# javieryu/nn_distributed_training

Measured on NVIDIA H100. Metric: consensus node-rounds/sec (DiNNO, dist_mnist_PAPER; rounds/sec x graph nodes), higher is better.
Workload: dtype fp64

## Files before the change

### nn_distributed_training_b200/ops/csrc/mnist_cl64.cu

```cuda
#include "mnist_device.cuh"

namespace nndt {
namespace mnist {

namespace cl64 {

constexpr int NT = 512, CL = 4, CELLS = 36, KC = 108, WS = 116, HS = 68;
constexpr int PXR = 10 * HW;
constexpr int KT = (KC + 7) / 8;
constexpr int HR = 68;
NNDT_DEVINL int hr(int j) { return (j >> 4) * 17 + (j & 15); }
constexpr int PART_WC = 0, PART_BC = 75, PART_B1 = 78, PART_W2 = 142, PART_B2 = 782, PART_LOSS = 792, PART_N = 793;

template <int MS>
struct Smem {
  static constexpr int NO = MS / CL;
  static constexpr bool kDoublePix = MS <= 32;
  static constexpr int PXS = kDoublePix ? PXR + 2 : PXR;
  double w[HID * WS];
  double a[MS * WS];
  double h[MS * HS];
  alignas(16) unsigned char img[kDoublePix ? MS * PXS * 8 : MS * PXS];
  double lut[kDoublePix ? 1 : 256];
  double h_loc[NO * HR > CL * 80 ? NO * HR : CL * 80];
  double dh_loc[NO * HID];
  double part[800];
  double w2[NCLS * HR];
  alignas(16) double b1[HID];
  alignas(16) double b2[16];
  double wc[80];
  double dz[NO * 16];
  double red[NO];
  int sidx[MS];
  int label[MS];
  float valid[MS];
  unsigned char arg[MS * KC];
};
static_assert(sizeof(Smem<16>) <= 227 * 1024 && sizeof(Smem<32>) <= 227 * 1024 && sizeof(Smem<64>) <= 227 * 1024,
              "shared memory budget");

NNDT_DEVINL double wmax(double v) {
#pragma unroll
  for (int o = 16; o > 0; o >>= 1) v = fmax(v, __shfl_xor_sync(0xffffffffu, v, o));
  return v;
}
template <int H>
NNDT_DEVINL void fold_half(double (&v)[16], int lane) {
  const bool up = (lane & (2 * H)) != 0;
#pragma unroll
  for (int i = 0; i < H; ++i) {
    const double send = up ? v[i] : v[i + H], keep = up ? v[i + H] : v[i];
    v[i] = keep + __shfl_xor_sync(0xffffffffu, send, 2 * H);
  }
}
NNDT_DEVINL void warp_reduce_scatter16(double (&v)[16], int lane) {
  fold_half<8>(v, lane); fold_half<4>(v, lane); fold_half<2>(v, lane); fold_half<1>(v, lane);
  v[0] += __shfl_xor_sync(0xffffffffu, v[0], 1);
}
NNDT_DEVINL void dmma_nv(double (&c)[4], double a0, double a1, double b) {
  asm("mma.sync.aligned.m16n8k4.row.col.f64.f64.f64.f64 {%0,%1,%2,%3}, {%4,%5}, {%6}, {%0,%1,%2,%3};"
      : "+d"(c[0]), "+d"(c[1]), "+d"(c[2]), "+d"(c[3])
      : "d"(a0), "d"(a1), "d"(b));
}
template <int NJ, int K, class FA, class FB>
NNDT_DEVINL void gemm_k(double (&c)[NJ][4], int m0, int n0, int lane, FA A, FB B) {
  static_assert(K % 4 == 0, "k steps of 4");
  const int g = lane >> 2, t = lane & 3;
  double a0 = A(m0 + g, t), a1 = A(m0 + g + 8, t), b[NJ];
#pragma unroll
  for (int j = 0; j < NJ; ++j) b[j] = B(t, n0 + 8 * j + g);
#pragma unroll
  for (int k0 = 0; k0 < K; k0 += 4) {
    double na0 = 0.0, na1 = 0.0, nb[NJ];
    if (k0 + 4 < K) {
      const int k = k0 + 4 + t;
      na0 = A(m0 + g, k); na1 = A(m0 + g + 8, k);
#pragma unroll
      for (int j = 0; j < NJ; ++j) nb[j] = B(k, n0 + 8 * j + g);
    }
#pragma unroll
    for (int j = 0; j < NJ; ++j) dmma_nv(c[j], a0, a1, b[j]);
    if (k0 + 4 < K) {
      a0 = na0; a1 = na1;
#pragma unroll
      for (int j = 0; j < NJ; ++j) b[j] = nb[j];
    }
  }
}
NNDT_DEVINL void stamp(long long* prof, int idx, int tid) {
  if (prof != nullptr && tid == 0) {
    long long t;
    asm volatile("mov.u64 %0, %%globaltimer;" : "=l"(t));
    prof[idx] = t;
  }
}

template <int MS>
__global__ void __cluster_dims__(CL, 1, 1) __launch_bounds__(NT, 1)
mnist_cl64_train_kernel(const Args a, const GenericShape gs) {
  using SM = Smem<MS>;
  constexpr int NO = SM::NO, PXS = SM::PXS;
  constexpr bool kDoublePix = SM::kDoublePix;
  static_assert(MS % 16 == 0 && NO <= NT / 32, "tile geometry");
  static_assert(CELLS % 2 == 0 && NCLS % 2 == 0 && 32 + NCLS / 2 <= NT, "16-byte parameter copies");
  extern __shared__ __align__(16) unsigned char smem_raw[];
  SM& sm = *reinterpret_cast<SM*>(smem_raw);
  const int tid = threadIdx.x, warp = tid >> 5, lane = tid & 31;
  const int l = blockIdx.z, bsplit = blockIdx.y, nsplit = gridDim.y;
  const int c = (int)cluster_rank();
  const double* th = reinterpret_cast<const double*>(a.theta) + (size_t)l * a.n_pad;
  const double pmean = gs.mean, pis = gs.inv_std;
  const bool u8 = a.x_is_u8 != 0;
  double* imgd = reinterpret_cast<double*>(sm.img);
  auto pix = [&](int s, int p) -> double {
    if constexpr (kDoublePix) return imgd[s * PXS + p];
    else if (u8) return sm.lut[sm.img[s * PXR + p]];
    else return (double)__ldg(reinterpret_cast<const float*>(a.x) + (size_t)sm.sidx[s] * 784 + 6 * HW * c + p);
  };
  long long* prof = a.prof != nullptr ? a.prof + ((l * nsplit + bsplit) * CL + c) * 64 : nullptr;
  stamp(prof, 0, tid);

  const int call = a.calls != nullptr ? a.calls[l] : 0;
  const BatchGeom bg = batch_geom<true>(a, l, call);
  if (tid < MS) {
    int idx = 0, lab = 0; float ok = 0.f;
    const uint32_t t = (uint32_t)(bsplit * MS + tid);
    if (t < bg.bs) {
      ok = 1.f;
      idx = a.direct ? (int)(l * a.batch + t) : bg.shard_off + (int)feistel_permute(bg.start + t, bg.m, bg.key);
      lab = (int)a.y[idx];
    }
    sm.sidx[tid] = idx; sm.valid[tid] = ok; sm.label[tid] = lab;
  }
  if constexpr (!kDoublePix)
    if (tid < 256) sm.lut[tid] = ((double)tid * (1.0 / 255.0) - pmean) * pis;
  __syncthreads();
  constexpr int NU8 = (MS * 35 + NT - 1) / NT, NF4 = kDoublePix ? (MS * 70 + NT - 1) / NT : 1;
  uint2 pu[NU8]; float4 pf[NF4];
  if (u8) {
#pragma unroll
    for (int i = 0; i < NU8; ++i) {
      const int o = tid + i * NT;
      pu[i] = make_uint2(0, 0);
      if (o < MS * 35) {
        const int s = o / 35, q = o - s * 35;
        if (sm.valid[s] != 0.f)
          pu[i] = *reinterpret_cast<const uint2*>(reinterpret_cast<const unsigned char*>(a.x) + (size_t)sm.sidx[s] * 784 + 6 * HW * c + 8 * q);
      }
    }
  } else if constexpr (kDoublePix) {
#pragma unroll
    for (int i = 0; i < NF4; ++i) {
      const int o = tid + i * NT;
      pf[i] = make_float4(0.f, 0.f, 0.f, 0.f);
      if (o < MS * 70) {
        const int s = o / 70, q = o - s * 70;
        if (sm.valid[s] != 0.f)
          pf[i] = *reinterpret_cast<const float4*>(reinterpret_cast<const float*>(a.x) + (size_t)sm.sidx[s] * 784 + 6 * HW * c + 4 * q);
      }
    }
  }
  if (u8) {
#pragma unroll
    for (int i = 0; i < NU8; ++i) {
      const int o = tid + i * NT;
      if (o < MS * 35) {
        const int s = o / 35, q = o - s * 35;
        if constexpr (kDoublePix) {
          const uint32_t w[2] = {pu[i].x, pu[i].y};
          double* dst = imgd + s * PXS + 8 * q;
#pragma unroll
          for (int j = 0; j < 8; ++j) dst[j] = ((double)((w[j >> 2] >> (8 * (j & 3))) & 0xff) * (1.0 / 255.0) - pmean) * pis;
        } else {
          *reinterpret_cast<uint2*>(sm.img + s * PXR + 8 * q) = pu[i];
        }
      }
    }
  } else if constexpr (kDoublePix) {
#pragma unroll
    for (int i = 0; i < NF4; ++i) {
      const int o = tid + i * NT;
      if (o < MS * 70) {
        double* dst = imgd + (o / 70) * PXS + 4 * (o % 70);
        dst[0] = pf[i].x; dst[1] = pf[i].y; dst[2] = pf[i].z; dst[3] = pf[i].w;
      }
    }
  }
  stamp(prof, 1, tid);
  pdl_wait();
  pdl_launch_dependents();
  stamp(prof, 2, tid);

  constexpr int NW2 = (NCLS * HID + NT - 1) / NT;
  double wcv = 0.0, w2v[NW2];
  if (tid < 75) wcv = __ldcg(th + a.off_wc + tid);
  else if (tid < 78) wcv = __ldcg(th + a.off_bc + (tid - 75));
#pragma unroll
  for (int i = 0; i < NW2; ++i) {
    const int o = tid + i * NT;
    w2v[i] = o < NCLS * HID ? __ldcg(th + a.off_w2 + o) : 0.0;
  }
  for (int o = tid; o < HID * KC / 2; o += NT) {
    const int j = o / (KC / 2), r = o - j * (KC / 2), ch = r / (CELLS / 2), q = 2 * (r - ch * (CELLS / 2));
    cp_async16(sm.w + j * WS + ch * CELLS + q, th + a.off_w1 + (size_t)j * FC1_IN + ch * NPOOL + CELLS * c + q);
  }
  if (tid < HID / 2) cp_async16(sm.b1 + 2 * tid, th + a.off_b1 + 2 * tid);
  else if (tid >= 32 && tid < 32 + NCLS / 2) cp_async16(sm.b2 + 2 * (tid - 32), th + a.off_b2 + 2 * (tid - 32));
  cp_async_commit();
  if (tid < 78) sm.wc[tid] = wcv;
#pragma unroll
  for (int i = 0; i < NW2; ++i) {
    const int o = tid + i * NT;
    if (o < NCLS * HID) sm.w2[(o / HID) * HR + hr(o % HID)] = w2v[i];
  }
  __syncthreads();
  stamp(prof, 3, tid);

  for (int it = tid; it < MS * CELLS; it += NT) {
    const int s = it / CELLS, cell = it - s * CELLS;
    const int pr = cell / PHW, px = cell - pr * PHW;
    const int p0 = (2 * pr) * HW + 2 * px;
    double patch[6][6];
    if constexpr (kDoublePix) {
      const double* src = imgd + s * PXS + p0;
#pragma unroll
      for (int r = 0; r < 6; ++r)
#pragma unroll
        for (int q = 0; q < 6; q += 2) {
          const double2 v = *reinterpret_cast<const double2*>(src + r * HW + q);
          patch[r][q] = v.x; patch[r][q + 1] = v.y;
        }
    } else {
#pragma unroll
      for (int r = 0; r < 6; ++r)
#pragma unroll
        for (int q = 0; q < 6; ++q) patch[r][q] = pix(s, p0 + r * HW + q);
    }
    const bool ok = sm.valid[s] != 0.f;
#pragma unroll 1
    for (int ch = 0; ch < F; ++ch) {
      double a00 = 0, a01 = 0, a10 = 0, a11 = 0;
#pragma unroll
      for (int ky = 0; ky < KS; ++ky)
#pragma unroll
        for (int kx = 0; kx < KS; ++kx) {
          const double w = sm.wc[ch * 25 + ky * 5 + kx];
          a00 += w * patch[ky][kx]; a01 += w * patch[ky][kx + 1];
          a10 += w * patch[ky + 1][kx]; a11 += w * patch[ky + 1][kx + 1];
        }
      double m = a00; int ai = 0;
      if (a01 > m) { m = a01; ai = 1; }
      if (a10 > m) { m = a10; ai = 2; }
      if (a11 > m) { m = a11; ai = 3; }
      m += sm.wc[75 + ch];
      m = (ok && m > 0.0) ? m : 0.0;
      sm.a[s * WS + ch * CELLS + cell] = m;
      sm.arg[s * KC + ch * CELLS + cell] = (unsigned char)(ai | (m > 0.0 ? 4 : 0));
    }
  }
  cp_async_wait<0>();
  __syncthreads();
  stamp(prof, 4, tid);

  {
    constexpr int NJ1 = MS == 64 ? 2 : 1, NGRP = 8 / NJ1;
    if (warp < (MS / 16) * NGRP) {
      const int m0 = 16 * (warp / NGRP), n0 = 8 * NJ1 * (warp % NGRP);
      double acc[NJ1][4];
      zero(acc);
      gemm_k<NJ1, KC>(acc, m0, n0, lane, at(sm.a, WS), at_t(sm.w, WS));
#pragma unroll
      for (int j = 0; j < NJ1; ++j)
#pragma unroll
        for (int i = 0; i < 4; ++i) sm.h[frow(m0, lane, i) * HS + fcol(n0 + 8 * j, lane, i)] = acc[j][i];
    }
  }
  stamp(prof, 5, tid);
  cluster_sync();
  stamp(prof, 6, tid);
  if (c == 0 && tid == 0 && a.calls != nullptr) {
    if (a.arrive == nullptr || nsplit == 1) a.calls[l] = call + 1;
    else if (atomicAdd(a.arrive + l, 1u) == (unsigned)nsplit - 1) { a.arrive[l] = 0; a.calls[l] = call + 1; }
  }

  const int s0 = c * NO;
  const double inv_bs = 1.0 / (double)(bg.bs ? bg.bs : 1);
  if (warp < NO) {
    const int sl = warp, s = s0 + sl;
    double hv[2];
#pragma unroll
    for (int q = 0; q < 2; ++q) {
      const int j = lane + 32 * q;
      const double* src = sm.h + s * HS + j;
      double v = sm.b1[j];
#pragma unroll
      for (int r = 0; r < CL; ++r) v += ld_dsmem(map_to(src, (uint32_t)r));
      hv[q] = v > 0.0 ? v : 0.0;
      sm.h_loc[sl * HR + hr(j)] = hv[q];
    }
    __syncwarp();
    double zp[2];
#pragma unroll
    for (int r = 0; r < 2; ++r) {
      const int o = lane + 32 * r, cc = o >> 2, part = o & 3;
      double v = 0.0;
      if (o < 4 * NCLS) {
#pragma unroll
        for (int jj = 0; jj < 16; ++jj) v += sm.h_loc[sl * HR + part * 17 + jj] * sm.w2[cc * HR + part * 17 + jj];
      }
      v += __shfl_xor_sync(0xffffffffu, v, 1);
      v += __shfl_xor_sync(0xffffffffu, v, 2);
      zp[r] = v;
    }
    static_assert(NCLS > 8 && NCLS <= 16, "two rounds of four lanes per class");
    const double z0 = __shfl_sync(0xffffffffu, zp[0], (4 * lane) & 31), z1 = __shfl_sync(0xffffffffu, zp[1], (4 * lane) & 31);
    const bool cls = lane < NCLS;
    const double zc = cls ? (lane < 8 ? z0 : z1) + sm.b2[lane] : -1.0e300;
    const double mx = wmax(zc);
    const double se = warp_sum(cls ? exp(zc - mx) : 0.0);
    const double lse = mx + log(se);
    const int y = sm.label[s];
    const double ok = (double)sm.valid[s];
    const double dzc = cls ? ok * inv_bs * (exp(zc - lse) - (lane == y ? 1.0 : 0.0)) : 0.0;
    if (cls) sm.dz[sl * 16 + lane] = dzc;
    if (lane == y) sm.red[sl] = ok * (lse - zc);
    double dh[2] = {0.0, 0.0};
#pragma unroll
    for (int cc = 0; cc < NCLS; ++cc) {
      const double d = __shfl_sync(0xffffffffu, dzc, cc);
      dh[0] += d * sm.w2[cc * HR + hr(lane)];
      dh[1] += d * sm.w2[cc * HR + hr(lane + 32)];
    }
#pragma unroll
    for (int q = 0; q < 2; ++q) sm.dh_loc[sl * HID + lane + 32 * q] = hv[q] > 0.0 ? dh[q] : 0.0;
  }
  __syncthreads();
  for (int o = tid; o < NCLS * HID; o += NT) {
    const int cc = o >> 6, j = o & 63;
    double v = 0.0;
    for (int sl = 0; sl < NO; ++sl) v += sm.dz[sl * 16 + cc] * sm.h_loc[sl * HR + hr(j)];
    sm.part[PART_W2 + o] = v;
  }
  if (tid < HID) {
    double v = 0.0;
    for (int sl = 0; sl < NO; ++sl) v += sm.dh_loc[sl * HID + tid];
    sm.part[PART_B1 + tid] = v;
  } else if (tid >= 64 && tid < 64 + NCLS) {
    double v = 0.0;
    for (int sl = 0; sl < NO; ++sl) v += sm.dz[sl * 16 + (tid - 64)];
    sm.part[PART_B2 + (tid - 64)] = v;
  } else if (tid == 96) {
    double v = 0.0;
    for (int sl = 0; sl < NO; ++sl) v += sm.red[sl];
    sm.part[PART_LOSS] = v * inv_bs;
  }
  stamp(prof, 7, tid);
  cluster_sync();
  stamp(prof, 8, tid);
  double* gp = reinterpret_cast<double*>(a.grad_part) + ((size_t)l * nsplit + bsplit) * a.n_pad;
  {
    constexpr int NE = PART_N - PART_B1, PER = (NE + CL - 1) / CL;
    const int o = PART_B1 + c * PER + tid;
    if (tid < PER && o < PART_N) {
      double v = 0.0;
#pragma unroll
      for (int r = 0; r < CL; ++r) v += ld_dsmem(map_to(sm.part + o, (uint32_t)r));
      if (o < PART_W2) gp[a.off_b1 + (o - PART_B1)] = v;
      else if (o < PART_B2) gp[a.off_w2 + (o - PART_W2)] = v;
      else if (o < PART_LOSS) gp[a.off_b2 + (o - PART_B2)] = v;
      else {
        a.loss_part[l * nsplit + bsplit] = (float)v;
        if (a.loss_mirror != nullptr) a.loss_mirror[l * nsplit + bsplit] = (float)v;
      }
    }
  }
  for (int o = tid; o < MS * HID; o += NT) {
    const int s = o >> 6, j = o & 63, r = s / NO;
    sm.h[s * HS + j] = ld_dsmem(map_to(sm.dh_loc + (s - r * NO) * HID + j, (uint32_t)r));
  }
  __syncthreads();
  stamp(prof, 9, tid);

  constexpr int NP2 = (MS / 16) * (KT / 2), NR2 = (NP2 + NT / 32 - 1) / (NT / 32);
  static_assert(KT % 2 == 0 && KC * MS + (NT / 32) * 16 <= HID * WS, "da1 and the conv-grad warp sums fit in the W slice");
  double acc2[NR2][2][4];
#pragma unroll
  for (int r = 0; r < NR2; ++r) {
    zero(acc2[r]);
    const int p = warp + r * (NT / 32);
    if (p < NP2) gemm_k<2, HID>(acc2[r], 16 * (p / (KT / 2)), 16 * (p % (KT / 2)), lane, at(sm.h, HS), at(sm.w, WS));
  }
  __syncthreads();
  stamp(prof, 10, tid);
  double* da1 = sm.w;
#pragma unroll
  for (int r = 0; r < NR2; ++r) {
    const int p = warp + r * (NT / 32);
    if (p < NP2) {
      const int m0 = 16 * (p / (KT / 2)), n0 = 16 * (p % (KT / 2));
#pragma unroll
      for (int jt = 0; jt < 2; ++jt)
#pragma unroll
        for (int i = 0; i < 4; ++i) {
          const int s = frow(m0, lane, i), k = fcol(n0 + 8 * jt, lane, i);
          if (k < KC) da1[k * MS + s] = (sm.arg[s * KC + k] & 4) ? acc2[r][jt][i] : 0.0;
        }
    }
  }
  __syncthreads();
  stamp(prof, 11, tid);
  constexpr int W3 = NT / 32 - HID / 16, NJ3 = KT / 2;
  if (warp >= W3) {
    const int m0 = 16 * (warp - W3);
#pragma unroll 1
    for (int n0 = 0; n0 < 8 * KT; n0 += 8 * NJ3) {
      double acc[NJ3][4];
      zero(acc);
      gemm_k<NJ3, MS>(acc, m0, n0, lane, at_t(sm.h, HS), at(sm.a, WS));
#pragma unroll
      for (int jt = 0; jt < NJ3; ++jt)
#pragma unroll
        for (int i = 0; i < 4; i += 2) {
          const int j = frow(m0, lane, i), k = fcol(n0 + 8 * jt, lane, i);
          if (k < KC) {
            const int ch = k / CELLS, cell = k - ch * CELLS;
            __stcg(reinterpret_cast<double2*>(gp + a.off_w1 + (size_t)j * FC1_IN + ch * NPOOL + CELLS * c + cell),
                   make_double2(acc[jt][i], acc[jt][i + 1]));
          }
        }
    }
    stamp(prof, 12, tid - W3 * 32);
  }
  constexpr int KW = 3, NRUN = MS * 3;
  static_assert(KS * KW < NT / 32 && F * KS <= 16, "conv-grad work split");
  double* wsums = sm.w + KC * MS;
  auto pix2 = [&](int s, int p) -> double2 {
    if constexpr (kDoublePix) return *reinterpret_cast<const double2*>(imgd + s * PXS + p);
    else return make_double2(pix(s, p), pix(s, p + 1));
  };
  if (warp < KS * KW) {
    const int ky = warp / KW;
    double acc[16];
#pragma unroll
    for (int i = 0; i < 16; ++i) acc[i] = 0.0;
#pragma unroll 1
    for (int r = tid - ky * KW * 32; r < NRUN; r += KW * 32) {
      const int s = r % MS, pr = r / MS;
      const int rb = (2 * pr + ky) * HW;
      double x0[6], x1[6];
#pragma unroll
      for (int px = 0; px < PHW; ++px) {
        const int p = rb + 2 * px;
        if (px == 0) {
#pragma unroll
          for (int q = 0; q < 6; q += 2) {
            const double2 u = pix2(s, p + q), v = pix2(s, p + HW + q);
            x0[q] = u.x; x0[q + 1] = u.y; x1[q] = v.x; x1[q + 1] = v.y;
          }
        } else {
#pragma unroll
          for (int q = 0; q < 4; ++q) { x0[q] = x0[q + 2]; x1[q] = x1[q + 2]; }
          const double2 u = pix2(s, p + 4), v = pix2(s, p + HW + 4);
          x0[4] = u.x; x0[5] = u.y; x1[4] = v.x; x1[5] = v.y;
        }
#pragma unroll
        for (int ch = 0; ch < F; ++ch) {
          const int k = ch * CELLS + pr * PHW + px;
          const double g = da1[k * MS + s];
          const int ai = sm.arg[s * KC + k] & 3;
          const double g00 = ai == 0 ? g : 0.0, g01 = ai == 1 ? g : 0.0, g10 = ai == 2 ? g : 0.0, g11 = ai == 3 ? g : 0.0;
#pragma unroll
          for (int kx = 0; kx < KS; ++kx) {
            double& t = acc[ch * KS + kx];
            t = fma(g00, x0[kx], t); t = fma(g01, x0[kx + 1], t);
            t = fma(g10, x1[kx], t); t = fma(g11, x1[kx + 1], t);
          }
        }
      }
    }
    warp_reduce_scatter16(acc, lane);
    if ((lane & 1) == 0 && (lane >> 1) < F * KS) wsums[warp * 16 + (lane >> 1)] = acc[0];
  } else if (warp == KS * KW) {
#pragma unroll 1
    for (int ch = 0; ch < F; ++ch) {
      double v = 0.0;
      for (int o = lane; o < CELLS * MS; o += 32) v += da1[ch * CELLS * MS + o];
      v = warp_sum(v);
      if (lane == 0) wsums[warp * 16 + ch] = v;
    }
  }
  __syncthreads();
  if (tid < 78) {
    double v = 0.0;
    if (tid < 75) {
      const int ch = tid / 25, t = tid - ch * 25, ky = t / KS, kx = t - ky * KS;
#pragma unroll
      for (int w = 0; w < KW; ++w) v += wsums[(ky * KW + w) * 16 + ch * KS + kx];
    } else {
      v = wsums[KS * KW * 16 + (tid - 75)];
    }
    st_dsmem(map_to(sm.h_loc + c * 80 + tid, 0u), v);
  }
  stamp(prof, 13, tid);
  cluster_sync();
  if (c == 0 && tid < 78) {
    double v = 0.0;
#pragma unroll
    for (int r = 0; r < CL; ++r) v += sm.h_loc[r * 80 + tid];
    gp[tid < 75 ? a.off_wc + tid : a.off_bc + (tid - 75)] = v;
  }
  stamp(prof, 14, tid);
}

template <int MS>
static cudaError_t prepare_ms() {
  static cudaError_t prep = cudaFuncSetAttribute(mnist_cl64_train_kernel<MS>, cudaFuncAttributeMaxDynamicSharedMemorySize, (int)sizeof(Smem<MS>));
  return prep;
}

template <int MS>
static cudaError_t launch_ms(const Args& a, const GenericShape& gs, cudaStream_t st) {
  const cudaError_t prep = prepare_ms<MS>();
  if (prep != cudaSuccess) return prep;
  cudaLaunchConfig_t cfg{};
  cfg.gridDim = dim3(CL, 64 / MS, a.L); cfg.blockDim = dim3(NT);
  cfg.dynamicSmemBytes = sizeof(Smem<MS>); cfg.stream = st;
  cudaLaunchAttribute attr[1];
  attr[0].id = cudaLaunchAttributeProgrammaticStreamSerialization;
  attr[0].val.programmaticStreamSerializationAllowed = 1;
  static const bool no_pdl = getenv("NNDT_NO_PDL") != nullptr;
  cfg.attrs = attr; cfg.numAttrs = no_pdl ? 0 : 1;
  return cudaLaunchKernelEx(&cfg, mnist_cl64_train_kernel<MS>, a, gs);
}

template <int MS>
static int max_clusters_ms() {
  if (prepare_ms<MS>() != cudaSuccess) { cudaGetLastError(); return 0; }
  cudaLaunchConfig_t cfg{};
  cfg.gridDim = dim3(CL, 1, 1); cfg.blockDim = dim3(NT); cfg.dynamicSmemBytes = sizeof(Smem<MS>);
  int n = 0;
  if (cudaOccupancyMaxActiveClusters(&n, mnist_cl64_train_kernel<MS>, &cfg) != cudaSuccess) { cudaGetLastError(); return 0; }
  return n;
}

}

cudaError_t launch_train_cl64(const Args& a, const GenericShape& gs, int nsplit, cudaStream_t st) {
  switch (nsplit) {
    case 1: return cl64::launch_ms<64>(a, gs, st);
    case 2: return cl64::launch_ms<32>(a, gs, st);
    case 4: return cl64::launch_ms<16>(a, gs, st);
  }
  return cudaErrorInvalidValue;
}

int cl64_max_active_clusters(int nsplit) {
  switch (nsplit) {
    case 1: return cl64::max_clusters_ms<64>();
    case 2: return cl64::max_clusters_ms<32>();
    case 4: return cl64::max_clusters_ms<16>();
  }
  return 0;
}

int cl64_cluster_ctas() { return cl64::CL; }

}
}
```

Baseline: 161,900.

## Restructure conv loop to stream patch rows, raise threads to 640

The conv/pool stage now streams the 6x6 input patch two rows at a time and accumulates all channels at once, instead of holding the full patch and looping over channels with no unroll. This cuts register pressure and repeated FMA chains per channel. The block size grows from 512 to 640 threads, which changes the warp counts available to every warp-partitioned GEMM phase. GEMM 3 also uses a fixed 2-tile width per pass, and the gradient pointer is recomputed lazily to shorten live ranges. The larger block and per-channel accumulators risk higher register use or lower occupancy.

Result: faster. 167,200, median of 6 (+3.3%).

```diff
diff --git a/nn_distributed_training_b200/ops/csrc/mnist_cl64.cu b/nn_distributed_training_b200/ops/csrc/mnist_cl64.cu
--- a/nn_distributed_training_b200/ops/csrc/mnist_cl64.cu
+++ b/nn_distributed_training_b200/ops/csrc/mnist_cl64.cu
@@ -5,7 +5,7 @@
 
 namespace cl64 {
 
-constexpr int NT = 512, CL = 4, CELLS = 36, KC = 108, WS = 116, HS = 68;
+constexpr int NT = 640, CL = 4, CELLS = 36, KC = 108, WS = 116, HS = 68;
 constexpr int PXR = 10 * HW;
 constexpr int KT = (KC + 7) / 8;
 constexpr int HR = 68;
@@ -220,34 +220,43 @@
     const int s = it / CELLS, cell = it - s * CELLS;
     const int pr = cell / PHW, px = cell - pr * PHW;
     const int p0 = (2 * pr) * HW + 2 * px;
-    double patch[6][6];
-    if constexpr (kDoublePix) {
-      const double* src = imgd + s * PXS + p0;
-#pragma unroll
-      for (int r = 0; r < 6; ++r)
+    auto patch_row = [&](double (&x)[6], int r) {
+      if constexpr (kDoublePix) {
+        const double* src = imgd + s * PXS + p0 + r * HW;
 #pragma unroll
         for (int q = 0; q < 6; q += 2) {
-          const double2 v = *reinterpret_cast<const double2*>(src + r * HW + q);
-          patch[r][q] = v.x; patch[r][q + 1] = v.y;
-        }
-    } else {
-#pragma unroll
-      for (int r = 0; r < 6; ++r)
-#pragma unroll
-        for (int q = 0; q < 6; ++q) patch[r][q] = pix(s, p0 + r * HW + q);
+          const double2 v = *reinterpret_cast<const double2*>(src + q);
+          x[q] = v.x; x[q + 1] = v.y;
+        }
+      } else {
+#pragma unroll
+        for (int q = 0; q < 6; ++q) x[q] = pix(s, p0 + r * HW + q);
+      }
+    };
+    double acc[F][4], x0[6], x1[6];
+#pragma unroll
+    for (int ch = 0; ch < F; ++ch)
+#pragma unroll
+      for (int i = 0; i < 4; ++i) acc[ch][i] = 0;
+    patch_row(x0, 0);
+#pragma unroll
+    for (int ky = 0; ky < KS; ++ky) {
+      patch_row(x1, ky + 1);
+#pragma unroll
+      for (int kx = 0; kx < KS; ++kx)
+#pragma unroll
+        for (int ch = 0; ch < F; ++ch) {
+          const double w = sm.wc[ch * 25 + ky * 5 + kx];
+          acc[ch][0] += w * x0[kx]; acc[ch][1] += w * x0[kx + 1];
+          acc[ch][2] += w * x1[kx]; acc[ch][3] += w * x1[kx + 1];
+        }
+#pragma unroll
+      for (int q = 0; q < 6; ++q) x0[q] = x1[q];
     }
     const bool ok = sm.valid[s] != 0.f;
-#pragma unroll 1
+#pragma unroll
     for (int ch = 0; ch < F; ++ch) {
-      double a00 = 0, a01 = 0, a10 = 0, a11 = 0;
-#pragma unroll
-      for (int ky = 0; ky < KS; ++ky)
-#pragma unroll
-        for (int kx = 0; kx < KS; ++kx) {
-          const double w = sm.wc[ch * 25 + ky * 5 + kx];
-          a00 += w * patch[ky][kx]; a01 += w * patch[ky][kx + 1];
-          a10 += w * patch[ky + 1][kx]; a11 += w * patch[ky + 1][kx + 1];
-        }
+      const double a00 = acc[ch][0], a01 = acc[ch][1], a10 = acc[ch][2], a11 = acc[ch][3];
       double m = a00; int ai = 0;
       if (a01 > m) { m = a01; ai = 1; }
       if (a10 > m) { m = a10; ai = 2; }
@@ -357,11 +366,12 @@
   stamp(prof, 7, tid);
   cluster_sync();
   stamp(prof, 8, tid);
-  double* gp = reinterpret_cast<double*>(a.grad_part) + ((size_t)l * nsplit + bsplit) * a.n_pad;
+  auto grad_row = [&]() { return reinterpret_cast<double*>(a.grad_part) + ((size_t)l * nsplit + bsplit) * a.n_pad; };
   {
     constexpr int NE = PART_N - PART_B1, PER = (NE + CL - 1) / CL;
     const int o = PART_B1 + c * PER + tid;
     if (tid < PER && o < PART_N) {
+      double* gp = grad_row();
       double v = 0.0;
 #pragma unroll
       for (int r = 0; r < CL; ++r) v += ld_dsmem(map_to(sm.part + o, (uint32_t)r));
@@ -409,8 +419,10 @@
   }
   __syncthreads();
   stamp(prof, 11, tid);
-  constexpr int W3 = NT / 32 - HID / 16, NJ3 = KT / 2;
+  constexpr int W3 = NT / 32 - HID / 16, NJ3 = 2;
+  static_assert(KT % NJ3 == 0, "GEMM 3 passes cover the column tiles");
   if (warp >= W3) {
+    double* gp = grad_row();
     const int m0 = 16 * (warp - W3);
 #pragma unroll 1
     for (int n0 = 0; n0 < 8 * KT; n0 += 8 * NJ3) {
@@ -504,6 +516,7 @@
   stamp(prof, 13, tid);
   cluster_sync();
   if (c == 0 && tid < 78) {
+    double* gp = grad_row();
     double v = 0.0;
 #pragma unroll
     for (int r = 0; r < CL; ++r) v += sm.h_loc[r * 80 + tid];
```
